# ax-le/nn-fac

Measured on NVIDIA B200. Metric: NMF outer iters/sec (HALS & MU beta=1) at 65536x8192 r=64, higher is better.
Workload: dtype f32

## Files before the change

### nn-fac_b200/csrc/tc_sweep.cu

```cuda
#include <stdlib.h>
#include <type_traits>

#include "common.cuh"
#include "tc_common.cuh"

namespace {

using bf16 = __nv_bfloat16;

#ifndef SWEEP_POSTER4
#define SWEEP_POSTER4 0
#endif
constexpr int BLK = 16;
constexpr int TILE = 128;
constexpr uint32_t PLANE_BYTES = TILE * 64 * sizeof(bf16);
constexpr int NPLANES = 3;
constexpr int XMAXW = 8;
constexpr int XMAXG = 160;

template <int RP, int MT, bool LAG>
struct Cfg {
  static_assert(MT * RP <= 256, "512 tensor-memory columns: RP residual + RP master columns per tile");
  static constexpr int NBLK = RP / BLK;
  static constexpr int KR = RP / 64;
  static constexpr int MAX_TILES = MT;
  static constexpr int UPD_THREADS = MAX_TILES * TILE;
  static constexpr bool POSTER = SWEEP_POSTER4 || !(RP == 64 && MT == 4);
  static constexpr int NTHREADS = UPD_THREADS + MAX_TILES * 32 + (POSTER ? 32 : 0);
  static constexpr int TMEM_PER_TILE = 2 * RP;
  static constexpr uint32_t G_ATOM_BYTES = RP * 128;
  static constexpr uint32_t G_PLANE_BYTES = KR * G_ATOM_BYTES;
  static constexpr int NSPEC = LAG ? NBLK : (RP == 64 ? 3 : 6);
  static constexpr int NSM = (LAG && RP == 128) ? 4 : 2;
  static constexpr uint32_t BK_EXTRA_BYTES = (NSM - 2) * (BLK * 4) * UPD_THREADS;
  static constexpr size_t SMEM = NPLANES * G_PLANE_BYTES + (size_t)MAX_TILES * NPLANES * PLANE_BYTES + BK_EXTRA_BYTES + 512;
  static constexpr int MBANKS = LAG ? 4 : 2;
};

template <int RP>
struct alignas(16) SweepConst {
  float nh[RP / BLK][BLK][BLK];
  float invd[RP];
  int has_zero_diag;
};
__constant__ SweepConst<64> c_sw64;
__constant__ SweepConst<128> c_sw128;
template <int RP>
__device__ __forceinline__ const SweepConst<RP>& csw() {
  if constexpr (RP == 64) return c_sw64; else return c_sw128;
}

template <int RP>
__global__ void sweep_prep_kernel(const float* __restrict__ G, int64_t ld_g, int r, SweepConst<RP>* out, unsigned* gen,
                                  unsigned long long* mail, size_t mail_count) {
  constexpr int NBLK = RP / BLK;
  __shared__ unsigned next_gen;
  if (threadIdx.x == 0) next_gen = (*gen + 1u) & 0xffffu;
  __syncthreads();
  if (next_gen == 0u) {
    for (size_t i = threadIdx.x; i < mail_count; i += blockDim.x) mail[i] = 0ull;
    __syncthreads();
  }
  if (threadIdx.x == 0) *gen = next_gen == 0u ? 1u : next_gen;
  for (int idx = threadIdx.x; idx < NBLK * BLK * BLK; idx += blockDim.x) {
    const int B = idx / (BLK * BLK), e = (idx / BLK) % BLK, e2 = idx % BLK;
    const int k = B * BLK + e, k2 = B * BLK + e2;
    const float d2 = k2 < r ? G[(int64_t)k2 * ld_g + k2] : 0.f;
    out->nh[B][e][e2] = (k < r && k2 < r && d2 != 0.f && e2 > e) ? -G[(int64_t)k2 * ld_g + k] * (1.f / d2) : 0.f;
  }
  for (int k = threadIdx.x; k < RP; k += blockDim.x) {
    const float d = k < r ? G[(int64_t)k * ld_g + k] : 0.f;
    out->invd[k] = d != 0.f ? 1.f / d : 0.f;
  }
  if (threadIdx.x == 0) {
    int z = 0;
    for (int k = 0; k < r; ++k) z |= (G[(int64_t)k * ld_g + k] == 0.f);
    out->has_zero_diag = z;
  }
}

struct TcSweepArgs {
  const float* b;
  const float* G;
  const float* Vin;
  float* V;
  int64_t ld_b, ld_g, ld_v, ld_vin, n;
  int nsplit;
  int64_t split_stride;
  bf16 *fh, *fl;
  bf16 *rowh, *rowl;
  int64_t ld_plane;
  int r_pad, row_pitch;
  int r, maxiter, cols_per_cta;
  double delta;
  float sp;
  unsigned long long* mail;
  const unsigned* gen;
  double* result;
  int xworld, xrank;
  unsigned xgen;
  unsigned long long* xboard[XMAXW];
  int xgrid[XMAXW];
};

using tc::tmem_st16;
using tc::tmem_st_wait;

__device__ __forceinline__ void named_bar_sync(int id, int nthreads) {
  asm volatile("bar.sync %0, %1;" ::"r"(id), "r"(nthreads) : "memory");
}

__device__ __forceinline__ uint32_t pack_bf16(float a, float b) {
  const __nv_bfloat162 p = __floats2bfloat162_rn(a, b);
  return *reinterpret_cast<const uint32_t*>(&p);
}

__device__ __forceinline__ void store_chunk(uint8_t* plane_hi, int row, int chunk, const float* x, uint32_t plane_stride) {
  uint32_t h[4], m[4], l[4];
#pragma unroll
  for (int i = 0; i < 4; ++i) {
    const float a = x[2 * i], b = x[2 * i + 1];
    h[i] = pack_bf16(a, b);
    const float a1 = a - __uint_as_float(h[i] << 16), b1 = b - __uint_as_float(h[i] & 0xffff0000u);
    m[i] = pack_bf16(a1, b1);
    const float a2 = a1 - __uint_as_float(m[i] << 16), b2 = b1 - __uint_as_float(m[i] & 0xffff0000u);
    l[i] = pack_bf16(a2, b2);
  }
  uint8_t* p = plane_hi + (uint32_t)row * 128u + (uint32_t)((chunk ^ (row & 7)) << 4);
  *reinterpret_cast<uint4*>(p) = make_uint4(h[0], h[1], h[2], h[3]);
  *reinterpret_cast<uint4*>(p + plane_stride) = make_uint4(m[0], m[1], m[2], m[3]);
  *reinterpret_cast<uint4*>(p + 2 * plane_stride) = make_uint4(l[0], l[1], l[2], l[3]);
}

__device__ __forceinline__ void store_chunk2(uint8_t* plane_hi, int row, int chunk, const float* x, uint32_t plane_stride) {
  uint32_t h[4], m[4];
#pragma unroll
  for (int i = 0; i < 4; ++i) {
    const float a = x[2 * i], b = x[2 * i + 1];
    h[i] = pack_bf16(a, b);
    m[i] = pack_bf16(a - __uint_as_float(h[i] << 16), b - __uint_as_float(h[i] & 0xffff0000u));
  }
  uint8_t* p = plane_hi + (uint32_t)row * 128u + (uint32_t)((chunk ^ (row & 7)) << 4);
  *reinterpret_cast<uint4*>(p) = make_uint4(h[0], h[1], h[2], h[3]);
  *reinterpret_cast<uint4*>(p + plane_stride) = make_uint4(m[0], m[1], m[2], m[3]);
}

__device__ __forceinline__ float warp_sum_f(float v) {
#pragma unroll
  for (int o = 16; o > 0; o >>= 1) v += __shfl_xor_sync(0xffffffffu, v, o);
  return v;
}

using tc::elect_one;

__device__ __forceinline__ unsigned long long ld_relaxed_u64(const unsigned long long* p) {
  unsigned long long v;
  asm volatile("ld.relaxed.gpu.global.u64 %0, [%1];" : "=l"(v) : "l"(p) : "memory");
  return v;
}
__device__ __forceinline__ void st_relaxed_u64(unsigned long long* p, unsigned long long v) {
  asm volatile("st.relaxed.gpu.global.u64 [%0], %1;" ::"l"(p), "l"(v) : "memory");
}
__device__ __forceinline__ unsigned long long ld_relaxed_sys_u64(const unsigned long long* p) {
  unsigned long long v;
  asm volatile("ld.relaxed.sys.global.u64 %0, [%1];" : "=l"(v) : "l"(p) : "memory");
  return v;
}
__device__ __forceinline__ void st_relaxed_sys_u64(unsigned long long* p, unsigned long long v) {
  asm volatile("st.relaxed.sys.global.u64 [%0], %1;" ::"l"(p), "l"(v) : "memory");
}

__device__ __forceinline__ void issue_step_update(uint64_t a_hi, uint64_t g_hi, uint32_t d, uint32_t idesc, uint64_t GP) {
  constexpr uint64_t AP = PLANE_BYTES >> 4;
  tc::umma_bf16(d, a_hi, g_hi, idesc, true);
  tc::umma_bf16(d, a_hi, g_hi + GP, idesc, true);
  tc::umma_bf16(d, a_hi + AP, g_hi, idesc, true);
}

__device__ __forceinline__ void issue_kslice(uint64_t a_hi, uint64_t g_hi, uint32_t d, uint32_t idesc, uint64_t GP) {
  constexpr uint64_t AP = PLANE_BYTES >> 4;
  tc::umma_bf16(d, a_hi, g_hi, idesc, true);
  tc::umma_bf16(d, a_hi, g_hi + GP, idesc, true);
  tc::umma_bf16(d, a_hi + AP, g_hi, idesc, true);
  tc::umma_bf16(d, a_hi, g_hi + 2 * GP, idesc, true);
  tc::umma_bf16(d, a_hi + AP, g_hi + GP, idesc, true);
  tc::umma_bf16(d, a_hi + 2 * AP, g_hi, idesc, true);
}

template <int B, int N>
struct BlockLoop {
  template <class F>
  static __device__ __forceinline__ void run(F& f) {
    f(std::integral_constant<int, B>{});
    BlockLoop<B + 1, N>::run(f);
  }
};
template <int N>
struct BlockLoop<N, N> {
  template <class F>
  static __device__ __forceinline__ void run(F&) {}
};

template <int RP, int MT, bool LAG>
__global__ void __launch_bounds__(Cfg<RP, MT, LAG>::NTHREADS, 1) tc_sweep_kernel(const TcSweepArgs a) {
  using C = Cfg<RP, MT, LAG>;
  constexpr int MAX_TILES = C::MAX_TILES, UPD_THREADS = C::UPD_THREADS, TMEM_PER_TILE = C::TMEM_PER_TILE, KR = C::KR;
  constexpr uint32_t G_PLANE_BYTES = C::G_PLANE_BYTES, G_ATOM_BYTES = C::G_ATOM_BYTES;
  constexpr uint64_t GP = G_PLANE_BYTES >> 4;
  extern __shared__ __align__(1024) uint8_t smem[];
  uint8_t* g_planes = smem;
  uint8_t* v_planes = smem + NPLANES * G_PLANE_BYTES;
  uint8_t* bk_extra = v_planes + (size_t)MAX_TILES * NPLANES * PLANE_BYTES;
  uint8_t* tail = bk_extra + C::BK_EXTRA_BYTES;
  uint64_t* s_full = reinterpret_cast<uint64_t*>(tail);
  uint64_t* s_ready = s_full + MAX_TILES;
  float* redf = reinterpret_cast<float*>(s_ready + MAX_TILES);
  uint32_t* tmem_slot = reinterpret_cast<uint32_t*>(redf + 48);
  volatile uint32_t* s_done = tmem_slot + 1;
  volatile uint32_t* s_quit = s_done + MAX_TILES;
  volatile uint32_t* s_posted = s_quit + 1;

  const int warp = threadIdx.x >> 5, lane = threadIdx.x & 31;
  const int r = a.r;
  const int nblk = (r + BLK - 1) / BLK;
  const int64_t cta_col0 = (int64_t)blockIdx.x * a.cols_per_cta;
  int64_t cta_cols = a.n - cta_col0;
  if (cta_cols > a.cols_per_cta) cta_cols = a.cols_per_cta;
  const int ntiles = (int)((cta_cols + TILE - 1) / TILE);

  if (warp == 0) {
    if (lane == 0) {
      for (int t = 0; t < MAX_TILES; ++t) {
        tc::mbar_init(&s_full[t], 1);
        tc::mbar_init(&s_ready[t], TILE);
      }
      for (int t = 0; t < MAX_TILES; ++t) s_done[t] = 0;
      *s_quit = 0;
      *s_posted = 0;
      tc::fence_barrier_init();
    }
    __syncwarp();
    tc::tmem_alloc(tmem_slot, 512);
  }
  if (threadIdx.x < UPD_THREADS) {
    for (int idx = threadIdx.x; idx < RP * (RP / 8); idx += UPD_THREADS) {
      const int j = idx / (RP / 8), c = idx % (RP / 8);
      const float dj = j < r ? a.G[(int64_t)j * a.ld_g + j] : 0.f;
      const float sj = dj != 0.f ? -1.f / dj : 0.f;
      float x[8];
#pragma unroll
      for (int i = 0; i < 8; ++i) {
        const int l = c * 8 + i;
        x[i] = (j < r && l < r) ? a.G[(int64_t)j * a.ld_g + l] * sj : 0.f;
      }
      store_chunk(g_planes + (c >> 3) * G_ATOM_BYTES, j, c & 7, x, G_PLANE_BYTES);
    }
  }
  tc::fence_proxy_async_smem();
  tc::tcgen05_fence_before();
  __syncthreads();
  tc::tcgen05_fence_after();
  const uint32_t tmem_base = *tmem_slot;
  const uint32_t idesc = tc::umma_idesc_bf16(TILE, RP);
  const uint64_t g_desc = tc::umma_desc_k_sw128(tc::smem_u32(g_planes));

  if (C::POSTER && warp == UPD_THREADS / 32 + MAX_TILES) {
    constexpr unsigned MB = C::MBANKS;
    const unsigned nb = gridDim.x;
    const unsigned gen = *a.gen;
    const bool collective = a.xworld > 0;
    for (unsigned e = 0;; ++e) {
      named_bar_sync(2, UPD_THREADS + 32);
      if (*s_quit) break;
      float sum = 0.f;
#pragma unroll
      for (int w = 0; w < UPD_THREADS / 32; ++w) sum += redf[(e & 1u) * 16 + w];
      const unsigned tag = collective ? ((a.xgen & 0xffffu) << 16) | (e + 1u) : (gen << 16) | (e + 1u);
      const unsigned long long bits = ((unsigned long long)tag << 32) | __float_as_uint(sum);
      if (collective) {
        const size_t xbank = (size_t)((a.xgen & 1u) * 4u + (e % MB)) * (XMAXW * XMAXG);
        if (lane < a.xworld) st_relaxed_sys_u64(a.xboard[lane] + xbank + (size_t)a.xrank * XMAXG + blockIdx.x, bits);
      } else if (nb > 1) {
        for (unsigned t = lane; t < nb; t += 32) st_relaxed_u64(a.mail + ((size_t)(e % MB) * nb + t) * nb + blockIdx.x, bits);
      }
      __syncwarp();
      if (lane == 0) *s_posted = e + 1u;
    }
  } else if (warp >= UPD_THREADS / 32) {
    const int tile = __shfl_sync(0xffffffffu, warp, 0) - UPD_THREADS / 32;
    if (tile < ntiles) {
      const uint64_t a_desc = tc::umma_desc_k_sw128(tc::smem_u32(v_planes + (size_t)tile * NPLANES * PLANE_BYTES));
      const uint32_t d = tmem_base + (uint32_t)(tile * TMEM_PER_TILE);
      uint32_t phase = 0;
      for (int kr = 0; kr < KR; ++kr) {
        if (kr * 4 >= nblk) break;
        tc::mbar_wait(&s_ready[tile], phase);
        phase ^= 1;
        tc::tcgen05_fence_after();
        if (elect_one()) {
          for (int ks = 0; ks < 4 && kr * 4 + ks < nblk; ++ks)
            issue_kslice(a_desc + (uint64_t)(ks * 2), g_desc + (uint64_t)(kr * (G_ATOM_BYTES >> 4) + ks * 2), d, idesc, GP);
          tc::umma_commit(&s_full[tile]);
        }
        __syncwarp();
      }
      for (int B = 0;; B = (B + 1 < nblk) ? B + 1 : 0) {
        tc::mbar_wait(&s_ready[tile], phase);
        phase ^= 1;
        if (s_done[tile]) break;
        tc::tcgen05_fence_after();
        if (elect_one()) {
          issue_step_update(a_desc + (uint64_t)((B & 3) * 2), g_desc + (uint64_t)((B >> 2) * (G_ATOM_BYTES >> 4) + (B & 3) * 2), d, idesc, GP);
          tc::umma_commit(&s_full[tile]);
        }
        __syncwarp();
      }
    }
  } else {
    const int tile = warp >> 2, q = warp & 3;
    const bool active = tile < ntiles;
    const int row = q * 32 + lane;
    const int64_t col = cta_col0 + (int64_t)tile * TILE + row;
    const bool valid = active && (int64_t)tile * TILE + row < cta_cols;
    uint8_t* vh = v_planes + (size_t)tile * NPLANES * PLANE_BYTES;
    const uint32_t t_w = tmem_base + ((uint32_t)(q * 32) << 16) + (uint32_t)(tile * TMEM_PER_TILE);
    const uint32_t t_v = t_w + RP;
    uint32_t s_phase = 0;

    if (active) {
#pragma unroll
      for (int c0 = 0; c0 < RP; c0 += 16) {
        uint32_t w[16];
        if (c0 < nblk * BLK) {
          float bv[16];
#pragma unroll
          for (int j = 0; j < 16; ++j) bv[j] = (valid && c0 + j < r) ? a.b[(int64_t)(c0 + j) * a.ld_b + col] : 0.f;
          for (int sp = 1; sp < a.nsplit; ++sp) {
            float t[16];
#pragma unroll
            for (int j = 0; j < 16; ++j)
              t[j] = (valid && c0 + j < r) ? a.b[(int64_t)sp * a.split_stride + (int64_t)(c0 + j) * a.ld_b + col] : 0.f;
#pragma unroll
            for (int j = 0; j < 16; ++j) bv[j] += t[j];
          }
#pragma unroll
          for (int j = 0; j < 16; ++j) w[j] = __float_as_uint((valid && c0 + j < r) ? (bv[j] - a.sp) * csw<RP>().invd[c0 + j] : 0.f);
        } else {
#pragma unroll
          for (int j = 0; j < 16; ++j) w[j] = 0u;
        }
        tmem_st16(t_w + c0, w);
      }
#pragma unroll
      for (int kr = 0; kr < KR; ++kr) {
        if (kr * 4 < nblk) {
          if (kr > 0) {
            tc::mbar_wait(&s_full[tile], s_phase);
            s_phase ^= 1;
          }
#pragma unroll
          for (int c1 = 0; c1 < 64; c1 += 16) {
            const int c0 = kr * 64 + c1;
            float x[16];
            uint32_t w[16];
#pragma unroll
            for (int j = 0; j < 16; ++j) x[j] = (valid && c0 + j < r) ? a.Vin[(int64_t)(c0 + j) * a.ld_vin + col] : 0.f;
#pragma unroll
            for (int j = 0; j < 16; ++j) w[j] = __float_as_uint(csw<RP>().invd[c0 + j] != 0.f ? x[j] : 0.f);
            tmem_st16(t_v + c0, w);
            store_chunk(vh, row, c1 / 8, &x[0], PLANE_BYTES);
            store_chunk(vh, row, c1 / 8 + 1, &x[8], PLANE_BYTES);
          }
          tmem_st_wait();
          tc::fence_proxy_async_smem();
          tc::tcgen05_fence_before();
          tc::mbar_arrive(&s_ready[tile]);
        } else {
          uint32_t z[16];
#pragma unroll
          for (int j = 0; j < 16; ++j) z[j] = 0u;
#pragma unroll
          for (int c1 = 0; c1 < 64; c1 += 16) tmem_st16(t_v + kr * 64 + c1, z);
          tmem_st_wait();
        }
      }
    }

    uint8_t* bkrow = vh + 2 * PLANE_BYTES + (uint32_t)row * 128u;
    uint8_t* bkrow2 = bk_extra + (uint32_t)(tile * TILE + row) * (uint32_t)((C::NSM - 2) * BLK * 4);
    (void)bkrow2;
#ifdef SWEEP_PROF
    long long prof[8] = {0, 0, 0, 0, 0, 0, 0, 0};
#define PROF_T(i) { const long long t__ = clock64(); prof[i] += t__ - tp; tp = t__; }
#define PROF_START long long tp = clock64();
#else
#define PROF_T(i)
#define PROF_START
#endif
    constexpr int NSM = C::NSM;
    uint32_t bkreg[C::NSPEC - NSM][BLK];
    auto block_update = [&](auto Bc, auto Backup) -> float {
      constexpr int B = decltype(Bc)::value;
      constexpr bool BACKUP = decltype(Backup)::value;
      float nd = 0.f;
      PROF_START
      uint32_t wb[BLK], keep[BLK];
      tc::tmem_ld16(t_v + B * BLK, keep);
      tc::mbar_wait(&s_full[tile], s_phase);
      s_phase ^= 1;
      tc::tcgen05_fence_after();
      PROF_T(0)
      tc::tmem_ld16(t_w + B * BLK, wb);
      tc::tmem_ld_wait();
      if (BACKUP && B < 2) {
#pragma unroll
        for (int c = 0; c < 4; ++c)
          *reinterpret_cast<uint4*>(bkrow + (((B * 4 + c) ^ (row & 7)) << 4)) = make_uint4(keep[4 * c], keep[4 * c + 1], keep[4 * c + 2], keep[4 * c + 3]);
      }
      if (BACKUP && B >= 2 && B < NSM) {
#pragma unroll
        for (int c = 0; c < 4; ++c)
          *reinterpret_cast<uint4*>(bkrow2 + ((((B - 2) * 4 + c) ^ (row & 7)) << 4)) = make_uint4(keep[4 * c], keep[4 * c + 1], keep[4 * c + 2], keep[4 * c + 3]);
      }
      if (BACKUP && B >= NSM && B < C::NSPEC) {
#pragma unroll
        for (int e = 0; e < BLK; ++e) bkreg[B >= NSM && B < C::NSPEC ? B - NSM : 0][e] = keep[e];
      }
      float u[BLK];
#pragma unroll
      for (int e = 0; e < BLK; ++e) u[e] = __uint_as_float(wb[e]);
      PROF_T(1)
      float dd[BLK];
      uint32_t vn[BLK];
#ifdef SWEEP_SCALAR_FMA
#pragma unroll
      for (int e = 0; e < BLK; ++e) {
        const float cur = __uint_as_float(keep[e]);
        const float d = fmaxf(u[e], -cur);
        if (e + 1 < BLK) u[e + 1] = fmaf(csw<RP>().nh[B][e][e + 1], d, u[e + 1]);
        dd[e] = d;
        vn[e] = __float_as_uint(cur + d);
        nd = fmaf(d, d, nd);
#pragma unroll
        for (int e2 = e + 2; e2 < BLK; ++e2) u[e2] = fmaf(csw<RP>().nh[B][e][e2], d, u[e2]);
      }
#else
#pragma unroll
      for (int e = 0; e < BLK; ++e) {
        const float cur = __uint_as_float(keep[e]);
        const float d = fmaxf(u[e], -cur);
        if (e + 1 < BLK) u[e + 1] = fmaf(csw<RP>().nh[B][e][e + 1], d, u[e + 1]);
        dd[e] = d;
        vn[e] = __float_as_uint(cur + d);
        nd = fmaf(d, d, nd);
        const float2 d2 = make_float2(d, d);
        constexpr int dummy = 0; (void)dummy;
        if (((e + 2) & 1) && e + 2 < BLK) u[e + 2] = fmaf(csw<RP>().nh[B][e][e + 2], d, u[e + 2]);
#pragma unroll
        for (int e2 = (e + 2 + 1) & ~1; e2 + 1 < BLK; e2 += 2) {
          const float2 c2 = *reinterpret_cast<const float2*>(&csw<RP>().nh[B][e][e2]);
          const float2 r2 = __ffma2_rn(c2, d2, make_float2(u[e2], u[e2 + 1]));
          u[e2] = r2.x; u[e2 + 1] = r2.y;
        }
      }
#endif
      PROF_T(2)
      tmem_st16(t_v + B * BLK, vn);
      store_chunk2(vh, row, 2 * (B & 3), &dd[0], PLANE_BYTES);
      store_chunk2(vh, row, 2 * (B & 3) + 1, &dd[8], PLANE_BYTES);
      PROF_T(3)
      tc::fence_proxy_async_smem();
      tmem_st_wait();
      tc::tcgen05_fence_before();
      tc::mbar_arrive(&s_ready[tile]);
      PROF_T(4)
      return nd;
    };

    float thr = 0.f, epsf = 1.f;
    int cnt = 1;
    unsigned epoch = 0;
    const unsigned nb = gridDim.x;
    const unsigned gen = *a.gen;
    const bool collective = a.xworld > 0;
    constexpr int NSPEC = C::NSPEC;
    int nspec = 0;
    float nd_spec = 0.f;
    std::integral_constant<bool, false> plain;
    std::integral_constant<bool, true> backup;
    constexpr unsigned MBANKS = C::MBANKS;
    unsigned nposts = 0;
    auto post = [&](float nd, unsigned e) {
      const float t = warp_sum_f(nd);
      ++nposts;
      if constexpr (C::POSTER) {
        if (lane == 0) {
          while (*s_posted < e) {}
          redf[(e & 1u) * 16 + warp] = t;
        }
        __syncwarp();
        asm volatile("bar.arrive 2, %0;" ::"n"(UPD_THREADS + 32) : "memory");
      } else {
        if (lane == 0) redf[(e & 1u) * 16 + warp] = t;
        named_bar_sync(1, UPD_THREADS);
        const unsigned tag = collective ? ((a.xgen & 0xffffu) << 16) | (e + 1u) : (gen << 16) | (e + 1u);
        if (collective ? threadIdx.x < (unsigned)a.xworld : (nb > 1 && threadIdx.x < nb)) {
          float sum = 0.f;
#pragma unroll
          for (int w = 0; w < UPD_THREADS / 32; ++w) sum += redf[(e & 1u) * 16 + w];
          const unsigned long long bits = ((unsigned long long)tag << 32) | __float_as_uint(sum);
          if (collective)
            st_relaxed_sys_u64(a.xboard[threadIdx.x] + (size_t)((a.xgen & 1u) * 4u + (e % MBANKS)) * (XMAXW * XMAXG) + (size_t)a.xrank * XMAXG + blockIdx.x, bits);
          else
            st_relaxed_u64(a.mail + ((size_t)(e % MBANKS) * nb + threadIdx.x) * nb + blockIdx.x, bits);
        }
      }
    };
    const bool poller = !collective && nb > 1 && threadIdx.x < nb;
    auto slot_of = [&](unsigned e) { return a.mail + ((size_t)(e % MBANKS) * nb + blockIdx.x) * nb + threadIdx.x; };
    constexpr int MAXE = (XMAXW * XMAXG + UPD_THREADS - 1) / UPD_THREADS;
    bool want[MAXE];
#pragma unroll
    for (int j = 0; j < MAXE; ++j) {
      const int en = threadIdx.x + j * UPD_THREADS;
      const int qr = en / XMAXG, c = en - qr * XMAXG;
      want[j] = collective && en < a.xworld * XMAXG && c < a.xgrid[qr < XMAXW ? qr : 0];
    }
    auto board_of = [&](unsigned e) { return a.xboard[a.xrank] + (size_t)((a.xgen & 1u) * 4u + (e % MBANKS)) * (XMAXW * XMAXG); };
    unsigned long long early_x[MAXE];
    auto peek = [&](unsigned e, unsigned long long& early) {
      if (poller) early = ld_relaxed_u64(slot_of(e));
      if (collective) {
        const unsigned long long* board = board_of(e);
#pragma unroll
        for (int j = 0; j < MAXE; ++j) early_x[j] = want[j] ? ld_relaxed_sys_u64(board + threadIdx.x + j * UPD_THREADS) : 0ull;
      }
    };
    auto collect = [&](unsigned e, unsigned long long early, bool peeked) -> float {
#ifdef SWEEP_PROF
      const long long tg0 = clock64();
#endif
      const unsigned tag = collective ? ((a.xgen & 0xffffu) << 16) | (e + 1u) : (gen << 16) | (e + 1u);
      float totf = 0.f;
      if (collective) {
        float got = 0.f;
        const unsigned long long* board = board_of(e);
        unsigned long long bits[MAXE];
#pragma unroll
        for (int j = 0; j < MAXE; ++j) bits[j] = peeked ? early_x[j] : (want[j] ? ld_relaxed_sys_u64(board + threadIdx.x + j * UPD_THREADS) : 0ull);
#pragma unroll
        for (int j = 0; j < MAXE; ++j) {
          if (want[j]) {
            uint32_t spins = 0;
            while ((unsigned)(bits[j] >> 32) != tag) {
              bits[j] = ld_relaxed_sys_u64(board + threadIdx.x + j * UPD_THREADS);
              if (++spins > (1u << 26)) __trap();
            }
            got += __uint_as_float((unsigned)bits[j]);
          }
        }
        got = warp_sum_f(got);
        if (lane == 0) redf[32 + warp] = got;
        named_bar_sync(1, UPD_THREADS);
#pragma unroll
        for (int w = 0; w < UPD_THREADS / 32; ++w) totf += redf[32 + w];
      } else if (nb > 1) {
        float got = 0.f;
        if (poller) {
          const unsigned long long* slot = slot_of(e);
          unsigned long long bits = peeked ? early : ld_relaxed_u64(slot);
          uint32_t spins = 0;
          while ((unsigned)(bits >> 32) != tag) {
            bits = ld_relaxed_u64(slot);
            if (++spins > (1u << 24)) __trap();
          }
          got = __uint_as_float((unsigned)bits);
        }
        got = warp_sum_f(got);
        if (lane == 0) redf[32 + warp] = got;
        named_bar_sync(1, UPD_THREADS);
#pragma unroll
        for (int w = 0; w < UPD_THREADS / 32; ++w) totf += redf[32 + w];
      } else {
        if (C::POSTER) named_bar_sync(1, UPD_THREADS);
#pragma unroll
        for (int w = 0; w < UPD_THREADS / 32; ++w) totf += redf[(e & 1u) * 16 + w];
      }
#ifdef SWEEP_PROF
      prof[6] += clock64() - tg0;
#endif
      return totf;
    };
    auto decide = [&](float totf) -> bool {
      if (cnt == 1) {
        const double thr_d = a.delta * (double)totf;
        thr = (float)thr_d;
        if ((double)thr < thr_d) thr = __uint_as_float(__float_as_uint(thr) + 1u);
      }
      epsf = totf;
      ++cnt;
      bool stop = !(epsf >= thr && cnt <= a.maxiter);
      if (totf == 0.f) {
        if (thr == 0.f && cnt < a.maxiter + 1) cnt = a.maxiter + 1;
        stop = true;
      }
      return stop;
    };
    if constexpr (LAG) {
      float nd = 0.f;
      if (active) {
        auto body = [&](auto Bc) {
          constexpr int B = decltype(Bc)::value;
          if (B < nblk) nd += block_update(Bc, plain);
        };
        BlockLoop<0, C::NBLK>::run(body);
      }
      post(nd, 0u);
      while (true) {
        unsigned long long early = 0ull;
        nspec = 0;
        if (cnt + 1 <= a.maxiter) {
          nspec = nblk;
          float nd2 = 0.f;
          auto spec = [&](auto Bc) {
            constexpr int B = decltype(Bc)::value;
            if (B < nblk) {
              if (B == nblk - 1) peek(epoch, early);
              if (active) nd2 += block_update(Bc, backup);
            }
          };
          BlockLoop<0, C::NBLK>::run(spec);
          post(nd2, epoch + 1u);
        }
        const float totf = collect(epoch, early, nspec > 0);
        ++epoch;
        if (decide(totf)) break;
      }
    } else {
    while (true) {
      float nd = nd_spec;
      if (active) {
        auto body = [&](auto Bc) {
          constexpr int B = decltype(Bc)::value;
          if (B < nblk && B >= nspec) nd += block_update(Bc, plain);
        };
        BlockLoop<0, C::NBLK>::run(body);
      }
      post(nd, epoch);
      unsigned long long early = 0ull;
      nspec = 0;
      nd_spec = 0.f;
      if (cnt + 1 <= a.maxiter) {
        nspec = nblk < NSPEC ? nblk : NSPEC;
        auto spec = [&](auto Bc) {
          constexpr int B = decltype(Bc)::value;
          if (B < nspec) {
            if (B == nspec - 1) peek(epoch, early);
            if (active) nd_spec += block_update(Bc, backup);
          }
        };
        BlockLoop<0, NSPEC>::run(spec);
      }
      const float totf = collect(epoch, early, nspec > 0);
      ++epoch;
      if (decide(totf)) break;
    }
    }
    if constexpr (C::POSTER) {
      if (lane == 0) {
        while (*s_posted < nposts) {}
        if (threadIdx.x == 0) *s_quit = 1;
      }
      __syncwarp();
      asm volatile("bar.arrive 2, %0;" ::"n"(UPD_THREADS + 32) : "memory");
    }
    if (active) {
      tc::mbar_wait(&s_full[tile], s_phase);
      tc::tcgen05_fence_after();
      if (lane == 0 && q == 0) s_done[tile] = 1;
      __threadfence_block();
      tc::mbar_arrive(&s_ready[tile]);
    }
    if (active) {
#pragma unroll
      for (int c0 = 0; c0 < RP; c0 += 16) {
        if (c0 < nblk * BLK) {
          uint32_t w[16];
          tc::tmem_ld16(t_v + c0, w);
          tc::tmem_ld_wait();
          if (c0 / BLK >= NSM && c0 / BLK < NSPEC && c0 / BLK < nspec) {
#pragma unroll
            for (int e = 0; e < BLK; ++e) w[e] = bkreg[c0 / BLK >= NSM && c0 / BLK < NSPEC ? c0 / BLK - NSM : 0][e];
          } else if (c0 / BLK >= 2 && c0 / BLK < NSM && c0 / BLK < nspec) {
#pragma unroll
            for (int c = 0; c < 4; ++c) {
              const uint4 b4 = *reinterpret_cast<const uint4*>(bkrow2 + ((((c0 / BLK - 2) * 4 + c) ^ (row & 7)) << 4));
              w[4 * c] = b4.x; w[4 * c + 1] = b4.y; w[4 * c + 2] = b4.z; w[4 * c + 3] = b4.w;
            }
          } else if (c0 / BLK < 2 && c0 / BLK < nspec) {
#pragma unroll
            for (int c = 0; c < 4; ++c) {
              const uint4 b4 = *reinterpret_cast<const uint4*>(bkrow + ((((c0 / BLK) * 4 + c) ^ (row & 7)) << 4));
              w[4 * c] = b4.x; w[4 * c + 1] = b4.y; w[4 * c + 2] = b4.z; w[4 * c + 3] = b4.w;
            }
          }
          float x[16];
#pragma unroll
          for (int j = 0; j < 16; ++j) {
            x[j] = __uint_as_float(w[j]);
            if (csw<RP>().has_zero_diag && valid && c0 + j < r && csw<RP>().invd[c0 + j] == 0.f) x[j] = a.Vin[(int64_t)(c0 + j) * a.ld_vin + col];
            if (valid && c0 + j < r) a.V[(int64_t)(c0 + j) * a.ld_v + col] = x[j];
          }
          if (a.fh != nullptr) {
            uint32_t hw[8], lw[8];
#pragma unroll
            for (int j = 0; j < 8; ++j) {
              const float p0 = (valid && c0 + 2 * j < r) ? x[2 * j] : 0.f, p1 = (valid && c0 + 2 * j + 1 < r) ? x[2 * j + 1] : 0.f;
              hw[j] = pack_bf16(p0, p1);
              lw[j] = pack_bf16(p0 - __uint_as_float(hw[j] << 16), p1 - __uint_as_float(hw[j] & 0xffff0000u));
            }
            if (valid) {
#pragma unroll
              for (int j = 0; j < 16; ++j) {
                if (c0 + j < a.r_pad) {
                  const uint32_t h = (j & 1) ? (hw[j >> 1] >> 16) : (hw[j >> 1] & 0xffffu), l = (j & 1) ? (lw[j >> 1] >> 16) : (lw[j >> 1] & 0xffffu);
                  reinterpret_cast<unsigned short*>(a.fh)[(int64_t)(c0 + j) * a.ld_plane + col] = (unsigned short)h;
                  reinterpret_cast<unsigned short*>(a.fl)[(int64_t)(c0 + j) * a.ld_plane + col] = (unsigned short)l;
                }
              }
              if (a.rowh != nullptr) {
                uint4* rh = reinterpret_cast<uint4*>(a.rowh + col * a.row_pitch + c0);
                uint4* rl = reinterpret_cast<uint4*>(a.rowl + col * a.row_pitch + c0);
                rh[0] = make_uint4(hw[0], hw[1], hw[2], hw[3]); rh[1] = make_uint4(hw[4], hw[5], hw[6], hw[7]);
                rl[0] = make_uint4(lw[0], lw[1], lw[2], lw[3]); rl[1] = make_uint4(lw[4], lw[5], lw[6], lw[7]);
              }
            }
          }
        }
      }
    }
#ifdef SWEEP_PROF
    if (blockIdx.x == 1 && (threadIdx.x == 0 || threadIdx.x == 32)) {
      printf("sweep prof (cycles/sweep) thr %d: mma_wait %lld tmem_ld %lld chain %lld split_store %lld fence_arrive %lld grid %lld\n",
             threadIdx.x, prof[0] / (cnt - 1), prof[1] / (cnt - 1), prof[2] / (cnt - 1), prof[3] / (cnt - 1), prof[4] / (cnt - 1),
             prof[6] / (cnt - 1));
    }
#endif
    if (blockIdx.x == 0 && threadIdx.x == 0) {
      a.result[0] = (double)epsf;
      a.result[1] = (double)cnt;
      a.result[2] = -1.0;
      a.result[3] = (double)(cnt - 1);
    }
  }
  tc::tcgen05_fence_before();
  __syncthreads();
  if (warp == 0) tc::tmem_dealloc(tmem_base, 512);
}

}

template <int RP, int MT, bool LAG>
static int sweep_launch(nnfac_ctx* ctx, TcSweepArgs& a, const float* UtU, int64_t ld_utu, int64_t grid, cudaStream_t st) {
  using C = Cfg<RP, MT, LAG>;
  void*& bank = ctx->sweep_const[RP == 64 ? 0 : 1];
  if (!bank) {
    if (RP == 64) NNFAC_CUDA(cudaGetSymbolAddress(&bank, c_sw64));
    else NNFAC_CUDA(cudaGetSymbolAddress(&bank, c_sw128));
  }
  unsigned* gen_dev = reinterpret_cast<unsigned*>(ctx->mail + ctx->mail_count);
  sweep_prep_kernel<RP><<<1, 256, 0, st>>>(UtU, ld_utu, a.r, (SweepConst<RP>*)bank, gen_dev, ctx->mail, ctx->mail_count);
  NNFAC_LAUNCH_CHECK(ctx);
  a.mail = ctx->mail; a.gen = gen_dev;
  NNFAC_CUDA(cudaFuncSetAttribute(tc_sweep_kernel<RP, MT, LAG>, cudaFuncAttributeMaxDynamicSharedMemorySize, (int)C::SMEM));
  void* params[] = {&a};
  NNFAC_CUDA(cudaLaunchCooperativeKernel((const void*)tc_sweep_kernel<RP, MT, LAG>, dim3((unsigned)grid), dim3(C::NTHREADS), params, C::SMEM, st));
  ctx->launches++;
  return NNFAC_OK;
}

int nnfac_tc_sweep_run(nnfac_ctx* ctx, const float* UtM, int64_t ld_utm, const float* UtU, int64_t ld_utu, const float* Vin,
                       int64_t ld_vin, float* V, int64_t ld_v, int r, int64_t n, int maxiter, double delta, double sparsity,
                       double* result, const nnfac_sweep_planes* planes, cudaStream_t st, int nsplit, int64_t split_stride) {
  if (r > 128 || maxiter < 1 || n < 1) return NNFAC_ERR_UNSUPPORTED;
  const int rp = r <= 64 ? 64 : 128;
  const int max_cols = (256 / rp) * TILE;
  int64_t cols = ceil_div64(n, ctx->sm_count);
  cols = ceil_div64(cols, 32) * 32;
  if (const char* force = getenv("NNFAC_SWEEP_COLS")) {
    const int64_t f = atoll(force);
    if (f >= 32 && f % 32 == 0 && f > cols) cols = f;
  }
  const nnfac_peer_group* pg = ctx->collective ? &ctx->peers : nullptr;
  if (pg) {
    int64_t widest = n;
    for (int q = 0; q < pg->world; ++q) if (ctx->collective_n[q] > widest) widest = ctx->collective_n[q];
    int64_t wc = ceil_div64(ceil_div64(widest, ctx->sm_count), 32) * 32;
    if (wc > max_cols) { nnfac_set_error("collective HALS solve: a slice of %lld columns at rank %d exceeds the tensor-core sweep", (long long)widest, r); return NNFAC_ERR_UNSUPPORTED; }
  }
  if (cols > max_cols) return NNFAC_ERR_UNSUPPORTED;
  const int64_t grid = ceil_div64(n, cols);
  if ((size_t)(4 * grid * grid) > ctx->mail_count || maxiter > 65000 || grid > XMAXG) return NNFAC_ERR_UNSUPPORTED;
  int rc = nnfac_guard_enter(ctx, NNFAC_GUARD_SWEEP, st);
  if (rc) return rc;
  TcSweepArgs a;
  a.b = UtM; a.G = UtU; a.Vin = Vin; a.V = V; a.ld_b = ld_utm; a.ld_g = ld_utu; a.ld_v = ld_v; a.ld_vin = ld_vin; a.n = n;
  a.r = r; a.maxiter = maxiter; a.cols_per_cta = (int)cols; a.delta = delta; a.sp = (float)sparsity;
  a.nsplit = nsplit > 0 ? nsplit : 1; a.split_stride = split_stride;
  a.fh = a.fl = a.rowh = a.rowl = nullptr; a.ld_plane = 0; a.r_pad = 0; a.row_pitch = 64;
  if (planes) {
    a.fh = (bf16*)planes->fh; a.fl = (bf16*)planes->fl; a.rowh = (bf16*)planes->rowh; a.rowl = (bf16*)planes->rowl;
    a.ld_plane = planes->ld_plane; a.r_pad = planes->r_pad; a.row_pitch = planes->row_pitch;
  }
  a.result = result;
  a.xworld = 0; a.xrank = 0; a.xgen = 0;
  for (int q = 0; q < XMAXW; ++q) { a.xboard[q] = nullptr; a.xgrid[q] = 0; }
  if (pg) {
    a.xworld = pg->world; a.xrank = pg->rank; a.xgen = ++ctx->collective_gen;
    for (int q = 0; q < pg->world; ++q) {
      a.xboard[q] = (unsigned long long*)pg->board[q];
      const int64_t nq = ctx->collective_n[q];
      int64_t cq = ceil_div64(ceil_div64(nq, ctx->sm_count), 32) * 32;
      a.xgrid[q] = nq > 0 ? (int)ceil_div64(nq, cq) : 0;
    }
    if (a.xgrid[pg->rank] != (int)grid) { nnfac_set_error("collective HALS solve: slice length %lld does not match the announced one", (long long)n); return NNFAC_ERR_ARG; }
  }
  static const int lag_env = [] { const char* e = getenv("NNFAC_SWEEP_LAG"); return e ? atoi(e) : 1; }();
  const int lag_mode = ctx->sweep_lag >= 0 ? ctx->sweep_lag : lag_env;
  int64_t decide_cols = cols;
  if (pg) {
    int64_t widest = n;
    for (int q = 0; q < pg->world; ++q) if (ctx->collective_n[q] > widest) widest = ctx->collective_n[q];
    decide_cols = ceil_div64(ceil_div64(widest, ctx->sm_count), 32) * 32;
  }
  const bool lag_possible = (pg != nullptr || grid > 1) && (rp == 128 || decide_cols <= 2 * TILE);
  const bool lag_pays = pg != nullptr || (decide_cols <= TILE && grid >= 64);
  const bool lag = lag_possible && (lag_mode >= 2 || (lag_mode == 1 && lag_pays));
  if (rp == 64) {
    if (lag) rc = sweep_launch<64, 2, true>(ctx, a, UtU, ld_utu, grid, st);
    else if (decide_cols <= 2 * TILE) rc = sweep_launch<64, 2, false>(ctx, a, UtU, ld_utu, grid, st);
    else rc = sweep_launch<64, 4, false>(ctx, a, UtU, ld_utu, grid, st);
  } else {
    rc = lag ? sweep_launch<128, 2, true>(ctx, a, UtU, ld_utu, grid, st) : sweep_launch<128, 2, false>(ctx, a, UtU, ld_utu, grid, st);
  }
  return rc;
}

int nnfac_tc_sweep_try(nnfac_ctx* ctx, const float* UtM, int64_t ld_utm, const float* UtU, int64_t ld_utu, float* V,
                       int64_t ld_v, int r, int64_t n, int maxiter, double delta, double sparsity, double* result,
                       cudaStream_t st) {
  return nnfac_tc_sweep_run(ctx, UtM, ld_utm, UtU, ld_utu, V, ld_v, V, ld_v, r, n, maxiter, delta, sparsity, result, nullptr, st, 1, 0);
}
```

Baseline: 779.5.

## Feed per-block step updates to UMMA from tensor memory instead of shared memory

When enough tensor-memory columns remain, each 16-column step delta is split into bf16 hi/lo halves and written into a dedicated TMEM region. The per-step MMA then reads its A operand from TMEM (the ts variant) rather than from swizzled shared-memory planes, which drops the smem stores and the async-proxy fence on the update critical path. The ready mbarrier also changes from one arrival per thread to one per warp, with expected counts sized to the valid warps in each tile, and warps with no valid rows now skip work entirely. This adds TMEM-operand descriptor and addressing assumptions, and changes the count logic for partial tiles.

```diff
diff --git a/nn-fac_b200/csrc/tc_sweep.cu b/nn-fac_b200/csrc/tc_sweep.cu
--- a/nn-fac_b200/csrc/tc_sweep.cu
+++ b/nn-fac_b200/csrc/tc_sweep.cu
@@ -33,6 +33,8 @@
   static constexpr int NSPEC = LAG ? NBLK : (RP == 64 ? 3 : 6);
   static constexpr int NSM = (LAG && RP == 128) ? 4 : 2;
   static constexpr uint32_t BK_EXTRA_BYTES = (NSM - 2) * (BLK * 4) * UPD_THREADS;
+  static constexpr uint32_t STEP_COL = MT * TMEM_PER_TILE;
+  static constexpr bool TS = STEP_COL + MT * BLK <= 512;
   static constexpr size_t SMEM = NPLANES * G_PLANE_BYTES + (size_t)MAX_TILES * NPLANES * PLANE_BYTES + BK_EXTRA_BYTES + 512;
   static constexpr int MBANKS = LAG ? 4 : 2;
 };
@@ -177,6 +179,12 @@
   tc::umma_bf16(d, a_hi + AP, g_hi, idesc, true);
 }
 
+__device__ __forceinline__ void issue_step_update_ts(uint32_t a_hi, uint64_t g_hi, uint32_t d, uint32_t idesc, uint64_t GP) {
+  tc::umma_bf16_ts(d, a_hi, g_hi, idesc, true);
+  tc::umma_bf16_ts(d, a_hi, g_hi + GP, idesc, true);
+  tc::umma_bf16_ts(d, a_hi + BLK / 2, g_hi, idesc, true);
+}
+
 __device__ __forceinline__ void issue_kslice(uint64_t a_hi, uint64_t g_hi, uint32_t d, uint32_t idesc, uint64_t GP) {
   constexpr uint64_t AP = PLANE_BYTES >> 4;
   tc::umma_bf16(d, a_hi, g_hi, idesc, true);
@@ -232,7 +240,8 @@
     if (lane == 0) {
       for (int t = 0; t < MAX_TILES; ++t) {
         tc::mbar_init(&s_full[t], 1);
-        tc::mbar_init(&s_ready[t], TILE);
+        const int64_t left = cta_cols - (int64_t)t * TILE;
+        tc::mbar_init(&s_ready[t], left >= TILE ? TILE / 32 : left > 0 ? (uint32_t)((left + 31) / 32) : TILE / 32);
       }
       for (int t = 0; t < MAX_TILES; ++t) s_done[t] = 0;
       *s_quit = 0;
@@ -291,6 +300,8 @@
     if (tile < ntiles) {
       const uint64_t a_desc = tc::umma_desc_k_sw128(tc::smem_u32(v_planes + (size_t)tile * NPLANES * PLANE_BYTES));
       const uint32_t d = tmem_base + (uint32_t)(tile * TMEM_PER_TILE);
+      const uint32_t a_step = tmem_base + C::STEP_COL + (uint32_t)(tile * BLK);
+      (void)a_step;
       uint32_t phase = 0;
       for (int kr = 0; kr < KR; ++kr) {
         if (kr * 4 >= nblk) break;
@@ -310,7 +321,9 @@
         if (s_done[tile]) break;
         tc::tcgen05_fence_after();
         if (elect_one()) {
-          issue_step_update(a_desc + (uint64_t)((B & 3) * 2), g_desc + (uint64_t)((B >> 2) * (G_ATOM_BYTES >> 4) + (B & 3) * 2), d, idesc, GP);
+          const uint64_t g = g_desc + (uint64_t)((B >> 2) * (G_ATOM_BYTES >> 4) + (B & 3) * 2);
+          if constexpr (C::TS) issue_step_update_ts(a_step, g, d, idesc, GP);
+          else issue_step_update(a_desc + (uint64_t)((B & 3) * 2), g, d, idesc, GP);
           tc::umma_commit(&s_full[tile]);
         }
         __syncwarp();
@@ -322,12 +335,15 @@
     const int row = q * 32 + lane;
     const int64_t col = cta_col0 + (int64_t)tile * TILE + row;
     const bool valid = active && (int64_t)tile * TILE + row < cta_cols;
+    const bool busy = __shfl_sync(0xffffffffu, valid, 0);
     uint8_t* vh = v_planes + (size_t)tile * NPLANES * PLANE_BYTES;
     const uint32_t t_w = tmem_base + ((uint32_t)(q * 32) << 16) + (uint32_t)(tile * TMEM_PER_TILE);
     const uint32_t t_v = t_w + RP;
+    const uint32_t t_step = tmem_base + ((uint32_t)(q * 32) << 16) + C::STEP_COL + (uint32_t)(tile * BLK);
+    (void)t_step;
     uint32_t s_phase = 0;
 
-    if (active) {
+    if (busy) {
 #pragma unroll
       for (int c0 = 0; c0 < RP; c0 += 16) {
         uint32_t w[16];
@@ -374,7 +390,8 @@
           tmem_st_wait();
           tc::fence_proxy_async_smem();
           tc::tcgen05_fence_before();
-          tc::mbar_arrive(&s_ready[tile]);
+          __syncwarp();
+          if (lane == 0) tc::mbar_arrive(&s_ready[tile]);
         } else {
           uint32_t z[16];
 #pragma unroll
@@ -466,13 +483,24 @@
 #endif
       PROF_T(2)
       tmem_st16(t_v + B * BLK, vn);
-      store_chunk2(vh, row, 2 * (B & 3), &dd[0], PLANE_BYTES);
-      store_chunk2(vh, row, 2 * (B & 3) + 1, &dd[8], PLANE_BYTES);
+      if constexpr (C::TS) {
+        uint32_t sw[BLK];
+#pragma unroll
+        for (int i = 0; i < BLK / 2; ++i) {
+          sw[i] = pack_bf16(dd[2 * i], dd[2 * i + 1]);
+          sw[BLK / 2 + i] = pack_bf16(dd[2 * i] - __uint_as_float(sw[i] << 16), dd[2 * i + 1] - __uint_as_float(sw[i] & 0xffff0000u));
+        }
+        tmem_st16(t_step, sw);
+      } else {
+        store_chunk2(vh, row, 2 * (B & 3), &dd[0], PLANE_BYTES);
+        store_chunk2(vh, row, 2 * (B & 3) + 1, &dd[8], PLANE_BYTES);
+      }
       PROF_T(3)
-      tc::fence_proxy_async_smem();
+      if constexpr (!C::TS) tc::fence_proxy_async_smem();
       tmem_st_wait();
       tc::tcgen05_fence_before();
-      tc::mbar_arrive(&s_ready[tile]);
+      __syncwarp();
+      if (lane == 0) tc::mbar_arrive(&s_ready[tile]);
       PROF_T(4)
       return nd;
     };
@@ -608,7 +636,7 @@
     };
     if constexpr (LAG) {
       float nd = 0.f;
-      if (active) {
+      if (busy) {
         auto body = [&](auto Bc) {
           constexpr int B = decltype(Bc)::value;
           if (B < nblk) nd += block_update(Bc, plain);
@@ -626,7 +654,7 @@
             constexpr int B = decltype(Bc)::value;
             if (B < nblk) {
               if (B == nblk - 1) peek(epoch, early);
-              if (active) nd2 += block_update(Bc, backup);
+              if (busy) nd2 += block_update(Bc, backup);
             }
           };
           BlockLoop<0, C::NBLK>::run(spec);
@@ -639,7 +667,7 @@
     } else {
     while (true) {
       float nd = nd_spec;
-      if (active) {
+      if (busy) {
         auto body = [&](auto Bc) {
           constexpr int B = decltype(Bc)::value;
           if (B < nblk && B >= nspec) nd += block_update(Bc, plain);
@@ -656,7 +684,7 @@
           constexpr int B = decltype(Bc)::value;
           if (B < nspec) {
             if (B == nspec - 1) peek(epoch, early);
-            if (active) nd_spec += block_update(Bc, backup);
+            if (busy) nd_spec += block_update(Bc, backup);
           }
         };
         BlockLoop<0, NSPEC>::run(spec);
@@ -674,14 +702,15 @@
       __syncwarp();
       asm volatile("bar.arrive 2, %0;" ::"n"(UPD_THREADS + 32) : "memory");
     }
-    if (active) {
+    if (busy) {
       tc::mbar_wait(&s_full[tile], s_phase);
       tc::tcgen05_fence_after();
       if (lane == 0 && q == 0) s_done[tile] = 1;
       __threadfence_block();
-      tc::mbar_arrive(&s_ready[tile]);
-    }
-    if (active) {
+      __syncwarp();
+      if (lane == 0) tc::mbar_arrive(&s_ready[tile]);
+    }
+    if (busy) {
 #pragma unroll
       for (int c0 = 0; c0 < RP; c0 += 16) {
         if (c0 < nblk * BLK) {
```

New measurement: 791.8 (median of 6 runs). 1.02x the previous value.
